# Tyler-Linchenwei/Graph-Distillation-for-Recommendation

Hardware: NVIDIA B200
Metric: kmeans_iters_per_s (higher is better)
Workload: dtype f32

## Files before the change

### graph-distillation-for-recommendation_b200/csrc/kmeans_tc.cu

```cuda
#include "tc_common.cuh"
#include <cuda.h>
#include <string.h>
#include <stdlib.h>

namespace gdr {

int launch_row_sqnorm(int64_t K, int D, const float* C, int64_t ldc, float* out, cudaStream_t s);
int launch_assign_simt_rows(int64_t max_rows, int64_t K, int64_t D, const float* X, int64_t ldx,
                            const float* CT, int64_t ldct, const float* cnorm, const int32_t* rows,
                            const int32_t* n_rows_dev, unsigned long long* packed, int32_t* labels,
                            const int32_t* labels_prev, int32_t* n_changed, float* best_out, cudaStream_t s);

constexpr int TC_BN = 128;
constexpr int TC_MAX_KB = 4;
constexpr int TC_BAR_KB = 5;
constexpr int TC_STAGES = 3;
constexpr int TC_THREADS = 320;
constexpr int TC_EPI_THREADS = 256;
constexpr int TC_TMEM_COLS = 256;
constexpr float TC_BAND = 3.0517578125e-05f;
static const int32_t* g_last_count1 = nullptr;
int g_tc_ablate = 0;
int g_tc_gate = 1;
extern int64_t g_topk_last_overflow;
// ... 780 lines not shown
          t1 = clock64();
          e_ld += t1 - t0;
        }
        tc_fence_before();
        mbar_arrive(&t_empty[a]);
        if (probe) e_ar += clock64() - t1;
      }
      if (half == 1) {
        s_merge[rl] = best;
        s_merge[128 + rl] = second;
        reinterpret_cast<int*>(s_merge)[256 + rl] = bidx;
      }
      asm volatile("bar.sync 1, %0;" ::"n"(TC_EPI_THREADS) : "memory");
      if (half == 0) {
        const float b1 = s_merge[rl], s1 = s_merge[128 + rl];
        const int i1 = reinterpret_cast<int*>(s_merge)[256 + rl];
        const float nb = fminf(best, b1);
        const float ns = fminf(fminf(second, s1), fmaxf(best, b1));
        const int ni = b1 < best ? i1 : bidx;
        if (row < N) {
          best_out[row] = nb;
          second_out[row] = ns;
          idx_out[row] = ni;
        }
      }
      asm volatile("bar.sync 1, %0;" ::"n"(TC_EPI_THREADS) : "memory");
    }
    if (probe && lane == 0) {
      g_ts_probe[7] = clock64() - e_tot;
      g_ts_probe[8] = e_wt;
      g_ts_probe[9] = e_ld;
      g_ts_probe[10] = e_ar;
      g_ts_probe[11] = e_st;
    }
  }
  tc_fence_before();
  __syncthreads();
  if (warp == 1) {
    __syncwarp();
    asm volatile("tcgen05.dealloc.cta_group::1.sync.aligned.b32 %0, %1;" ::"r"(tmem_base), "r"(512) : "memory");
  }
}

__device__ __forceinline__ uint32_t cluster_ctarank() {
  uint32_t r;
  asm volatile("mov.u32 %0, %%cluster_ctarank;" : "=r"(r));
  return r;
}
__device__ __forceinline__ void cluster_sync_all() {
  asm volatile("barrier.cluster.arrive.release.aligned;" ::: "memory");
  asm volatile("barrier.cluster.wait.acquire.aligned;" ::: "memory");
}
__device__ __forceinline__ uint32_t mapa_u32(uint32_t smem_addr, uint32_t cta_rank) {
  uint32_t r;
  asm volatile("mapa.shared::cluster.u32 %0, %1, %2;" : "=r"(r) : "r"(smem_addr), "r"(cta_rank));
  return r;
}
__device__ __forceinline__ void mbar_arrive_cluster(uint32_t cluster_addr) {
  asm volatile("mbarrier.arrive.release.cluster.shared::cluster.b64 _, [%0];" ::"r"(cluster_addr) : "memory");
}
__device__ __forceinline__ void tma_load_2d_2sm(void* smem_dst, const CUtensorMap* map, int c0, int c1,
                                                uint32_t bar_cluster_addr) {
  asm volatile(
      "cp.async.bulk.tensor.2d.cta_group::2.shared::cluster.global.mbarrier::complete_tx::bytes [%0], [%1, {%2, %3}], [%4];"
      ::"r"(smem_u32(smem_dst)), "l"(reinterpret_cast<uint64_t>(map)), "r"(c0), "r"(c1), "r"(bar_cluster_addr)
      : "memory");
}
__device__ __forceinline__ void tc_commit_2sm(uint64_t* bar, uint16_t cta_mask) {
  asm volatile(
      "tcgen05.commit.cta_group::2.mbarrier::arrive::one.shared::cluster.multicast::cluster.b64 [%0], %1;"
      ::"r"(smem_u32(bar)), "h"(cta_mask)
      : "memory");
}
__device__ __forceinline__ void tc_mma_tf32_2sm(uint32_t tmem_d, uint64_t adesc, uint64_t bdesc, uint32_t idesc,
                                                uint32_t accumulate) {
  asm volatile(
      "{\n\t.reg .pred p;\n\t"
      "setp.ne.b32 p, %4, 0;\n\t"
      "tcgen05.mma.cta_group::2.kind::tf32 [%0], %1, %2, %3, p;\n\t}"
      ::"r"(tmem_d), "l"(adesc), "l"(bdesc), "r"(idesc), "r"(accumulate)
      : "memory");
}

struct Tc2Cfg {
  static constexpr int BN = 256;
  static constexpr int kStageBytes = (BN / 2) * TC_BK * 4;
  static constexpr int kStages = 8;
  static constexpr int kTmemCols = 2 * BN;
  static constexpr int kTail = 512;
  __host__ __device__ static constexpr int x_blk(int kb) { return kb * TC_KBLK_BYTES; }
  __host__ __device__ static constexpr int c_stage(int nkb, int s) { return nkb * TC_KBLK_BYTES + s * kStageBytes; }
  __host__ __device__ static constexpr int bars(int nkb) { return c_stage(nkb, kStages); }
  __host__ __device__ static constexpr int total(int nkb) { return bars(nkb) + kTail + 1024; }
};

__global__ void __launch_bounds__(TC_THREADS, 1)
k_assign_tc_pair(const __grid_constant__ CUtensorMap map_x, const __grid_constant__ CUtensorMap map_c,
                 int64_t N_host, const int32_t* __restrict__ n_rows_dev, int D, int n_col_tiles, int nkb,
                 float* __restrict__ best_out, float* __restrict__ second_out, int32_t* __restrict__ idx_out, int ablate,
                 int fwd ) {
  using Cfg = Tc2Cfg;
  constexpr int S = Cfg::kStages;
  constexpr int BN = Cfg::BN;
  extern __shared__ uint8_t smem_raw[];
  uint8_t* smem = reinterpret_cast<uint8_t*>((reinterpret_cast<uintptr_t>(smem_raw) + 1023) & ~uintptr_t(1023));
  uint64_t* bars = reinterpret_cast<uint64_t*>(smem + Cfg::bars(nkb));
  uint64_t* x_full = bars;
  uint64_t* x_empty = bars + TC_BAR_KB;
  uint64_t* c_full = bars + 2 * TC_BAR_KB;
  uint64_t* c_empty = c_full + S;
  uint64_t* t_full = c_empty + S;
  uint64_t* t_empty = t_full + 2;
  uint64_t* c_peer = t_empty + 2;
  uint64_t* x_peer = c_peer + S;
  uint32_t* tmem_base_smem = reinterpret_cast<uint32_t*>(x_peer + TC_BAR_KB);

  const int warp = threadIdx.x >> 5;
  const int lane = threadIdx.x & 31;
  const uint32_t crank = cluster_ctarank();
  const bool leader = crank == 0;
  const int64_t N = n_rows_dev ? (int64_t)n_rows_dev[0] : N_host;
  const int n_row_tiles = (int)((N + TC_BM - 1) / TC_BM);
  const int n_units = (n_row_tiles + 1) / 2;
  const int unit0 = (int)blockIdx.x >> 1, unit_stride = (int)gridDim.x >> 1;

  if (warp == 0 && lane == 0) {
    for (int i = 0; i < TC_BAR_KB; ++i) {
      mbar_init(&x_full[i], 1);
      mbar_init(&x_empty[i], 1);
    }
    for (int i = 0; i < S; ++i) {
      mbar_init(&c_full[i], 1);
      mbar_init(&c_empty[i], 1);
    }
    for (int i = 0; i < 2; ++i) {
      mbar_init(&t_full[i], 1);
      mbar_init(&t_empty[i], 16);
    }
    for (int i = 0; i < S; ++i) mbar_init(&c_peer[i], 1);
    for (int i = 0; i < TC_BAR_KB; ++i) mbar_init(&x_peer[i], 1);
    asm volatile("fence.mbarrier_init.release.cluster;" ::: "memory");
  }
  if (warp == 1) {
    asm volatile("tcgen05.alloc.cta_group::2.sync.aligned.shared::cta.b32 [%0], %1;" ::"r"(smem_u32(tmem_base_smem)),
                 "r"(Cfg::kTmemCols)
                 : "memory");
    asm volatile("tcgen05.relinquish_alloc_permit.cta_group::2.sync.aligned;" ::: "memory");
  }
  tc_fence_before();
  __syncthreads();
  cluster_sync_all();
  tc_fence_after();
  const uint32_t tmem_base = *tmem_base_smem;

  if (warp == 0) {
    uint32_t tile_it = 0;
    int s = 0;
    uint32_t ph = 0;
    const uint32_t x_full0 = mapa_u32(smem_u32(&x_full[0]), 0), c_full0 = mapa_u32(smem_u32(&c_full[0]), 0);
    for (int un = unit0; un < n_units; un += unit_stride, ++tile_it) {
      const int rt = 2 * un + (int)crank;
      for (int kb = 0; kb < nkb; ++kb) {
        mbar_wait(&x_empty[kb], (tile_it & 1) ^ 1);
        if (elect_one()) {
          if (fwd) {
            mbar_expect_tx(&x_full[kb], TC_KBLK_BYTES);
            tma_load_2d(smem + Cfg::x_blk(kb), &map_x, kb * TC_BK, rt * TC_BM, &x_full[kb]);
          } else {
            if (leader) mbar_expect_tx(&x_full[kb], 2 * TC_KBLK_BYTES);
            tma_load_2d_2sm(smem + Cfg::x_blk(kb), &map_x, kb * TC_BK, rt * TC_BM, x_full0 + 8u * (uint32_t)kb);
          }
        }
        __syncwarp();
      }
      for (int ct = 0; ct < n_col_tiles; ++ct) {
        for (int kb = 0; kb < nkb; ++kb) {
          if (ablate >= 6) continue;
          mbar_wait(&c_empty[s], ph ^ 1);
          if (elect_one()) {
            if (ablate == 5) {
              if (leader || fwd) mbar_arrive(&c_full[s]);
            } else if (fwd) {
              mbar_expect_tx(&c_full[s], Cfg::kStageBytes);
              tma_load_2d(smem + Cfg::c_stage(nkb, s), &map_c, kb * TC_BK, ct * BN + (int)crank * (BN / 2), &c_full[s]);
            } else {
              if (leader) mbar_expect_tx(&c_full[s], 2 * Cfg::kStageBytes);
              tma_load_2d_2sm(smem + Cfg::c_stage(nkb, s), &map_c, kb * TC_BK, ct * BN + (int)crank * (BN / 2),
                              c_full0 + 8u * (uint32_t)s);
            }
          }
          __syncwarp();
          if (++s == S) {
            s = 0;
            ph ^= 1;
          }
        }
      }
    }
  } else if (warp == 1) {
    if (leader) {
      constexpr uint32_t idesc = umma_idesc_tf32(2 * TC_BM, BN);
      uint32_t tile_it = 0, g = 0;
      int s = 0;
      uint32_t ph = 0;
      const uint64_t dx0 = umma_desc_sw128(smem_u32(smem));
      const uint64_t dc0 = umma_desc_sw128(smem_u32(smem + Cfg::c_stage(nkb, 0)));
      constexpr uint64_t kKb = TC_KBLK_BYTES >> 4, kStage = Cfg::kStageBytes >> 4;
      for (int un = unit0; un < n_units; un += unit_stride, ++tile_it) {
        for (int ct = 0; ct < n_col_tiles; ++ct, ++g) {
          const uint32_t a = g & 1, aph = (g >> 1) & 1;
          if (ablate != 8) mbar_wait(&t_empty[a], aph ^ 1);
          tc_fence_after();
          const uint32_t tmem_d = tmem_base + a * BN;
          const bool last_ct = ct == n_col_tiles - 1;
          for (int kb = 0; kb < nkb; ++kb) {
            if (ct == 0) {
              mbar_wait(&x_full[kb], tile_it & 1);
              if (fwd) mbar_wait(&x_peer[kb], tile_it & 1);
            }
            if (ablate < 6) {
              mbar_wait(&c_full[s], ph);
              if (fwd) mbar_wait(&c_peer[s], ph);
            }
            tc_fence_after();
            const uint64_t d_x = dx0 + (uint64_t)kb * kKb;
            const uint64_t d_c = dc0 + (uint64_t)s * kStage;
            const int ksteps = min(TC_BK / 8, (D - kb * TC_BK + 7) >> 3);
            if (elect_one()) {
              if (ablate != 3 && ablate != 4 && ksteps == 4) {
#pragma unroll
                for (int k = 0; k < 4; ++k) {
                  const uint64_t adv = (uint64_t)((k * 8 * 4) >> 4);
                  tc_mma_tf32_2sm(tmem_d, d_x + adv, d_c + adv, idesc, (kb | k) != 0);
                }
              } else {
                for (int k = 0; k < ((ablate == 3 || (ablate == 4 && kb > 0)) ? 0 : ksteps); ++k) {
                  const uint64_t adv = (uint64_t)((k * 8 * 4) >> 4);
                  tc_mma_tf32_2sm(tmem_d, d_x + adv, d_c + adv, idesc, (kb | k) != 0);
                }
              }
              if (ablate < 6) tc_commit_2sm(&c_empty[s], 3);
              if (last_ct) tc_commit_2sm(&x_empty[kb], 3);
              if (kb == nkb - 1 && ablate != 8) tc_commit_2sm(&t_full[a], 3);
            }
            __syncwarp();
            if (++s == S) {
              s = 0;
              ph ^= 1;
            }
          }
        }
      }
    } else if (fwd) {
      uint32_t tile_it = 0;
      int s = 0;
      uint32_t ph = 0;
      const uint32_t c_peer0 = mapa_u32(smem_u32(&c_peer[0]), 0), x_peer0 = mapa_u32(smem_u32(&x_peer[0]), 0);
      for (int un = unit0; un < n_units; un += unit_stride, ++tile_it) {
        for (int ct = 0; ct < n_col_tiles; ++ct) {
          for (int kb = 0; kb < nkb; ++kb) {
            if (ct == 0) {
              mbar_wait(&x_full[kb], tile_it & 1);
              if (elect_one()) mbar_arrive_cluster(x_peer0 + 8u * (uint32_t)kb);
              __syncwarp();
            }
            mbar_wait(&c_full[s], ph);
            if (elect_one()) mbar_arrive_cluster(c_peer0 + 8u * (uint32_t)s);
            __syncwarp();
            if (++s == S) {
              s = 0;
              ph ^= 1;
            }
          }
        }
      }
    }
  } else {
    const int quarter = warp & 3;
    const int half = (warp - 2) >> 2;
    const int rl = quarter * 32 + lane;
    const uint32_t t_empty_leader[2] = {mapa_u32(smem_u32(&t_empty[0]), 0), mapa_u32(smem_u32(&t_empty[1]), 0)};
    __shared__ float s_mb[3][TC_BM];
    uint32_t g = 0;
    for (int un = unit0; un < (ablate == 8 ? 0 : n_units); un += unit_stride) {
      const int rt = 2 * un + (int)crank;
      const int64_t row = (int64_t)rt * TC_BM + rl;
      float best = INFINITY, second = INFINITY;
      int bidx = 0;
      for (int ct = 0; ct < n_col_tiles; ++ct, ++g) {
        const uint32_t a = g & 1, aph = (g >> 1) & 1;
        mbar_wait(&t_full[a], aph);
        tc_fence_after();
#pragma unroll 1
        for (int h2 = 0; h2 < (ablate == 2 ? 0 : BN / 128); ++h2) {
          const int col0 = half * (BN / 2) + h2 * 64;
          const uint32_t taddr = tmem_base + ((uint32_t)(quarter * 32) << 16) + a * BN + col0;
          uint32_t v[2][32];
          tc_ld_32x32(taddr, v[0]);
          tc_ld_32x32(taddr + 32, v[1]);
          tc_wait_ld();
#pragma unroll
          for (int c = 0; c < 2; ++c) {
            const int jbase = ct * BN + col0 + c * 32;
#pragma unroll
            for (int u0 = 0; u0 < 32; u0 += 8) {
              float m = fmaxf(fmaxf(__uint_as_float(v[c][u0]), __uint_as_float(v[c][u0 + 1])),
                              fmaxf(__uint_as_float(v[c][u0 + 2]), __uint_as_float(v[c][u0 + 3])));
              m = fmaxf(m, fmaxf(fmaxf(__uint_as_float(v[c][u0 + 4]), __uint_as_float(v[c][u0 + 5])),
                                 fmaxf(__uint_as_float(v[c][u0 + 6]), __uint_as_float(v[c][u0 + 7]))));
              if (__any_sync(0xffffffffu, -m < second)) {
#pragma unroll
                for (int u = u0; u < u0 + 8; ++u) {
                  const float d = -__uint_as_float(v[c][u]);
                  second = fminf(second, fmaxf(d, best));
                  bidx = d < best ? jbase + u : bidx;
                  best = fminf(best, d);
                }
              }
            }
          }
        }
        tc_fence_before();
        __syncwarp();
        if (lane == 0) mbar_arrive_cluster(t_empty_leader[a]);
      }
      if (half == 1) {
        s_mb[0][rl] = best;
        s_mb[1][rl] = second;
        reinterpret_cast<int*>(s_mb[2])[rl] = bidx;
      }
      asm volatile("bar.sync 1, %0;" ::"n"(TC_EPI_THREADS) : "memory");
      if (half == 0) {
        const float b1 = s_mb[0][rl], s1 = s_mb[1][rl];
        const int i1 = reinterpret_cast<int*>(s_mb[2])[rl];
        const float nb = fminf(best, b1);
        const float ns = fminf(fminf(second, s1), fmaxf(best, b1));
        const int ni = b1 < best ? i1 : bidx;
        if (row < N) {
          best_out[row] = nb;
          second_out[row] = ns;
          idx_out[row] = ni;
        }
      }
      asm volatile("bar.sync 1, %0;" ::"n"(TC_EPI_THREADS) : "memory");
    }
  }
  tc_fence_before();
  __syncthreads();
  cluster_sync_all();
  if (warp == 1) {
    asm volatile("tcgen05.dealloc.cta_group::2.sync.aligned.b32 %0, %1;" ::"r"(tmem_base), "r"(Cfg::kTmemCols) : "memory");
  }
}

__global__ void __launch_bounds__(128, 1) k_mma_probe_pair(int iters, long long* __restrict__ cycles) {
  extern __shared__ uint8_t smem_raw[];
  uint8_t* smem = reinterpret_cast<uint8_t*>((reinterpret_cast<uintptr_t>(smem_raw) + 1023) & ~uintptr_t(1023));
  __shared__ uint64_t bar;
  __shared__ uint32_t tmem_slot;
  for (int i = threadIdx.x; i < 8 * 128 * 128 / 4; i += blockDim.x) reinterpret_cast<float*>(smem)[i] = 0.f;
  const bool leader = cluster_ctarank() == 0;
  if (threadIdx.x == 0) {
    mbar_init(&bar, 1);
    asm volatile("fence.mbarrier_init.release.cluster;" ::: "memory");
  }
  if (threadIdx.x < 32) {
    asm volatile("tcgen05.alloc.cta_group::2.sync.aligned.shared::cta.b32 [%0], %1;" ::"r"(smem_u32(&tmem_slot)), "r"(512) : "memory");
    asm volatile("tcgen05.relinquish_alloc_permit.cta_group::2.sync.aligned;" ::: "memory");
  }
  asm volatile("fence.proxy.async.shared::cta;" ::: "memory");
  tc_fence_before();
  __syncthreads();
  cluster_sync_all();
  tc_fence_after();
  const uint32_t tmem_base = tmem_slot;
  if (leader && threadIdx.x < 32) {
    constexpr uint32_t idesc = umma_idesc_tf32(256, 256);
    const long long t0 = clock64();
    int issued = 0;
    for (int t = 0; issued < iters; ++t) {
      const uint32_t d = tmem_base + (uint32_t)(t & 1) * 256u;
      for (int kb = 0; kb < 4; ++kb) {
        const uint64_t da = umma_desc_sw128(smem_u32(smem + kb * 16384));
        const uint64_t db = umma_desc_sw128(smem_u32(smem + 65536 + ((t * 4 + kb) & 3) * 16384));
        const int ks = kb < 3 ? 4 : 1;
        tc_fence_after();
        if (elect_one()) {
          for (int k = 0; k < ks; ++k) {
            const uint64_t adv = (uint64_t)((k * 32) >> 4);
            tc_mma_tf32_2sm(d, da + adv, db + adv, idesc, (kb | k) != 0);
          }
        }
        __syncwarp();
        issued += ks;
      }
    }
    if (elect_one()) tc_commit_2sm(&bar, 1);
    __syncwarp();
    mbar_wait(&bar, 0);
    if (threadIdx.x == 0) cycles[0] = clock64() - t0;
  }
  tc_fence_before();
  __syncthreads();
  cluster_sync_all();
  if (threadIdx.x < 32) {
    asm volatile("tcgen05.dealloc.cta_group::2.sync.aligned.b32 %0, %1;" ::"r"(tmem_base), "r"(512) : "memory");
  }
}

__global__ void __launch_bounds__(256) k_tc_select1(int64_t N, const float* __restrict__ best,
                                                    const float* __restrict__ second,
                                                    const int32_t* __restrict__ idx,
                                                    const float* __restrict__ xnorm, const float* __restrict__ xdnorm,
                                                    const float* __restrict__ cnorm,
                                                    const float* __restrict__ cnorm_sqrt,
                                                    const float* __restrict__ cdnorm,
                                                    const float* __restrict__ cmax, float band,
// ... 418 lines not shown
         ws_need(2 * N, 4) + ws_need(2 * N * TC_CAND_CAP, 8)  + ws_need(N, 4)  +
         256  + 256;
}

template <int NPASS, int BN, int SUB>
static int launch_assign_tc(const CUtensorMap& m_xhi, const CUtensorMap& m_xlo, const CUtensorMap& m_chi,
                            const CUtensorMap& m_clo, int64_t N_max, const int32_t* n_rows_dev, int D_eff, int64_t Kp,
                            int nkb, const float* cnorm, float* best, float* second, int32_t* idx, cudaStream_t s,
                            TcGate gate = TcGate{nullptr, nullptr, nullptr, nullptr, 0.f}) {
  using Cfg = TcCfg<NPASS, BN, SUB>;
  static PerDevice<bool> attr_set_dev;
  bool& attr_set = attr_set_dev.get();
  if (!attr_set) {
    GDR_CUDA(cudaFuncSetAttribute(k_assign_tc<NPASS, BN, SUB>, cudaFuncAttributeMaxDynamicSharedMemorySize,
                                  TC_SMEM_LIMIT));
    attr_set = true;
  }
  int sms = kSMs;
  {
    int dev = 0;
    cudaGetDevice(&dev);
    cudaDeviceGetAttribute(&sms, cudaDevAttrMultiProcessorCount, dev);
  }
  const int64_t tiles = cdiv(N_max, TC_BM * SUB);
  const int grid = (int)(tiles < sms ? tiles : sms);
  k_assign_tc<NPASS, BN, SUB><<<grid, TC_THREADS, Cfg::total(nkb), s>>>(m_xhi, m_xlo, m_chi, m_clo, N_max, n_rows_dev, D_eff,
                                                                  (int)(Kp / BN), nkb, cnorm, best, second, idx, g_tc_ablate, gate);
  GDR_LAUNCHED();
  return GDR_OK;
}

static int launch_tc_cand(const CUtensorMap& m_x1, const CUtensorMap& m_c1, int64_t N_max, const int32_t* n_rows_dev,
                          int D_eff, int64_t Kp, int nkb, TcGate gate, TcCand cand, cudaStream_t s) {
  using Cfg = TcCfg<1, 256, 1>;
  static PerDevice<bool> attr_set_dev;
  bool& attr_set = attr_set_dev.get();
  if (!attr_set) {
    GDR_CUDA(cudaFuncSetAttribute(k_tc_cand, cudaFuncAttributeMaxDynamicSharedMemorySize, TC_SMEM_LIMIT));
    attr_set = true;
  }
  int sms = kSMs;
  {
    int dev = 0;
    cudaGetDevice(&dev);
    cudaDeviceGetAttribute(&sms, cudaDevAttrMultiProcessorCount, dev);
  }
  const int64_t tiles = cdiv(N_max, TC_BM);
  const int grid = (int)(tiles < sms ? tiles : sms);
  k_tc_cand<<<grid, TC_THREADS, Cfg::total(nkb), s>>>(m_x1, m_c1, N_max, n_rows_dev, D_eff, (int)(Kp / 256), nkb, gate, cand);
  GDR_LAUNCHED();
  return GDR_OK;
}

template <int BN>
static int launch_assign_tc_ts(const float* x1, int ldx1, const CUtensorMap& m_c, int64_t N_max, const int32_t* n_rows_dev,
                               int D_eff, int n_col_tiles, int nkb, float* best, float* second, int32_t* idx, cudaStream_t s,
                               TcGate gate) {
  using Cfg = TsCfg<BN>;
  static PerDevice<bool> attr_set_dev;
  bool& attr_set = attr_set_dev.get();
  if (!attr_set) {
    GDR_CUDA(cudaFuncSetAttribute(k_assign_tc_ts<BN>, cudaFuncAttributeMaxDynamicSharedMemorySize, TC_SMEM_LIMIT));
    attr_set = true;
  }
  int sms = kSMs;
  {
    int dev = 0;
    cudaGetDevice(&dev);
    cudaDeviceGetAttribute(&sms, cudaDevAttrMultiProcessorCount, dev);
  }
  const int64_t tiles = cdiv(N_max, TC_BM);
  const int grid = (int)(tiles < sms ? tiles : sms);
  k_assign_tc_ts<BN><<<grid, TC_THREADS, Cfg::total(), s>>>(x1, ldx1, m_c, N_max, n_rows_dev, D_eff, n_col_tiles, nkb, best,
                                                          second, idx, g_tc_ablate, gate);
  GDR_LAUNCHED();
  return GDR_OK;
}

__global__ void k_pad_aug(float* __restrict__ aug, int64_t r0, int64_t r1, int Dp1, int D) {
  const int64_t i = (int64_t)blockIdx.x * blockDim.x + threadIdx.x, n = (r1 - r0) * Dp1;
  if (i < n) aug[r0 * Dp1 + i] = (int)(i % Dp1) == D + 2 ? to_tf32(-1e30f) : 0.f;
}

static int launch_assign_tc_pair(const CUtensorMap& m_x, const CUtensorMap& m_c, int64_t N_max, const int32_t* n_rows_dev,
                                 int D_eff, int64_t Kp, int nkb, float* best, float* second, int32_t* idx, int fwd,
                                 cudaStream_t s) {
  static PerDevice<bool> attr_set_dev;
  bool& attr_set = attr_set_dev.get();
  if (!attr_set) {
    GDR_CUDA(cudaFuncSetAttribute(k_assign_tc_pair, cudaFuncAttributeMaxDynamicSharedMemorySize, Tc2Cfg::total(TC_BAR_KB)));
    attr_set = true;
  }
  int sms = kSMs;
  {
    int dev = 0;
    cudaGetDevice(&dev);
    cudaDeviceGetAttribute(&sms, cudaDevAttrMultiProcessorCount, dev);
  }
  const int64_t units = cdiv(cdiv(N_max, TC_BM), 2);
  const int pairs = (int)(units < sms / 2 ? units : sms / 2);
  cudaLaunchConfig_t cfg = {};
  cfg.gridDim = dim3(2 * pairs);
  cfg.blockDim = dim3(TC_THREADS);
  cfg.dynamicSmemBytes = Tc2Cfg::total(nkb);
  cfg.stream = s;
  cudaLaunchAttribute attr[1];
  attr[0].id = cudaLaunchAttributeClusterDimension;
  attr[0].val.clusterDim.x = 2;
  attr[0].val.clusterDim.y = 1;
  attr[0].val.clusterDim.z = 1;
  cfg.attrs = attr;
  cfg.numAttrs = 1;
  GDR_CUDA(cudaLaunchKernelEx(&cfg, k_assign_tc_pair, m_x, m_c, N_max, n_rows_dev, D_eff, (int)(Kp / Tc2Cfg::BN), nkb, best,
                              second, idx, g_tc_ablate, fwd));
  GDR_LAUNCHED();
  return GDR_OK;
}

int kmeans_assign_tc_run(int64_t N, int64_t K, int64_t D, const float* X, int64_t ldx, const void* xsplit,
                         const float* C, int64_t ldc, int32_t* labels, const int32_t* labels_prev,
                         int32_t* n_changed_dev, float* best_out, int32_t* n_refined_dev, void* ws,
                         int64_t ws_bytes, cudaStream_t s, const int32_t* labels_hint) {
  if (D > TC_MAX_KB * TC_BK) {
    set_error("kmeans_assign(tc): D=%lld > %d is not supported by the tensor-core path", (long long)D,
              TC_MAX_KB * TC_BK);
    return GDR_EUNSUPPORTED;
  }
  if (N >= (1ll << 31) - TC_BM || K >= (1ll << 31) - TC_KPAD) {
    set_error("kmeans_assign(tc): N or K exceeds int32 tile coordinates");
    return GDR_ERANGE;
  }
  const int Dp = dpad(D), Dp1 = dpad1(D);
  const int nkb = Dp / TC_BK, nkb1 = Dp1 / TC_BK;
  const int64_t Kp = align_up(K, TC_KPAD);
  XSplit xs = carve_xsplit(const_cast<void*>(xsplit), N, D);
  Workspace W(ws, ws_bytes);
  float* c_hi = W.take<float>(Kp * Dp);
  float* c_lo = W.take<float>(Kp * Dp);
  float* c_t = W.take<float>(Kp * Dp);
  float* c1 = W.take<float>((Kp + TC_TS_BN) * Dp1);
  float* cnorm = W.take<float>(Kp);
  float* cnorm_sqrt = W.take<float>(Kp);
  float* cdnorm = W.take<float>(Kp);
  float* cmax = W.take<float>(2);
  float* best = W.take<float>(N);
  float* second = W.take<float>(N);
  int32_t* idx = W.take<int32_t>(N);
  int32_t* amb_list = W.take<int32_t>(N);
  unsigned long long* amb_packed = W.take<unsigned long long>(N);
  int32_t* amb_count_ws = W.take<int32_t>(1);
  int32_t* list1 = W.take<int32_t>(N);
  int32_t* count1 = W.take<int32_t>(1);
  float* g_hi = W.take<float>(N * Dp);
  float* g_lo = W.take<float>(N * Dp);
  float* g_norm = W.take<float>(N);
  float* g_dnorm = W.take<float>(N);
  float* g_seed = W.take<float>(N);
  int32_t* cand_n = W.take<int32_t>(2 * N);
  int2* cand_list = W.take<int2>(2 * N * TC_CAND_CAP);
  int32_t* list2 = W.take<int32_t>(N);
  int32_t* cand_ctr = W.take<int32_t>(TC_CAND_CTRS);
  int32_t* amb_count = n_refined_dev ? n_refined_dev : amb_count_ws;
  if (!W.ok()) {
    set_error("kmeans_assign(tc): workspace too small");
    return GDR_EWORKSPACE;
  }
  const bool two_level = tc_two_level(N, best_out != nullptr);
  k_split_tf32<<<(unsigned)cdiv(Kp * 32, 256), 256, 0, s>>>(K, Kp, (int)D, Dp, C, ldc, c_hi, c_lo, nullptr, c_t, cnorm,
                                                           two_level ? c1 : nullptr, Dp1, 2, cdnorm);
  GDR_LAUNCHED();
  int rc;
  k_cnorm_finish<<<1, 1024, 0, s>>>(K, Kp, cnorm, two_level ? cdnorm : nullptr, cnorm_sqrt, cmax, amb_count, count1,
                                    two_level ? cand_ctr : nullptr, TC_CAND_CTRS);
  GDR_LAUNCHED();

  CUtensorMap m_xhi, m_xlo, m_chi, m_clo;
  if ((rc = make_map(&m_chi, c_hi, Kp, Dp, 128))) return rc;
  if ((rc = make_map(&m_clo, c_lo, Kp, Dp, 128))) return rc;

  if (!two_level) {
    if ((rc = make_map(&m_xhi, xs.hi, N, Dp, TC_BM))) return rc;
    if ((rc = make_map(&m_xlo, xs.lo, N, Dp, TC_BM))) return rc;
    {
      ProfileScope prof(PROF_ASSIGN, s);
      if ((rc = launch_assign_tc<3, 128, 1>(m_xhi, m_xlo, m_chi, m_clo, N, nullptr, (int)D, Kp, nkb, cnorm, best, second,
                                         idx, s)))
        return rc;
    }
    k_tc_select<<<(unsigned)cdiv(N, 256), 256, 0, s>>>(N, best, second, idx, xs.norm, cmax, TC_BAND, labels,
                                                      labels_prev, n_changed_dev, best_out, amb_list, amb_count,
                                                      amb_packed);
    GDR_LAUNCHED();
  } else {
    ProfileScope prof(PROF_ASSIGN, s);
    CUtensorMap m_x1, m_c1;
    bool cand_level = false;
    if ((rc = make_map(&m_x1, xs.x1, N, Dp1, TC_BM))) return rc;
    if (g_tc_screen == 2) {
      if ((rc = make_map(&m_c1, c1, Kp, Dp1, 128))) return rc;
      if ((rc = launch_assign_tc<1, 128, 2>(m_x1, m_x1, m_c1, m_c1, N, nullptr, (int)D + TC_AUG, Kp, nkb1, cnorm, best, second,
                                         idx, s)))
        return rc;
    } else if (g_tc_screen == 4 || g_tc_screen == 5) {
      if ((rc = make_map(&m_c1, c1, Kp, Dp1, 128))) return rc;
      if ((rc = launch_assign_tc_pair(m_x1, m_c1, N, nullptr, (int)D + TC_AUG, Kp, nkb1, best, second, idx,
                                      g_tc_screen == 5 ? 1 : 0, s)))
        return rc;
    } else {
      const int ka = (int)align_up(D + TC_AUG, 8);
      const int ts_bn = (g_tc_screen == 6 && ka <= 512 - 2 * TC_TS_BN) ? TC_TS_BN : 0;
      cand_level = g_tc_cand != 0 && ts_bn == 0;
      const int64_t k_rows = ts_bn == TC_TS_BN ? align_up(K, TC_TS_BN) : Kp;
      if (k_rows > Kp) {
        k_pad_aug<<<(unsigned)cdiv((k_rows - Kp) * Dp1, 256), 256, 0, s>>>(c1, Kp, k_rows, Dp1, (int)D);
        GDR_LAUNCHED();
      }
      if ((rc = make_map(&m_c1, c1, std::max(Kp, k_rows), Dp1, ts_bn ? ts_bn : 256))) return rc;
      TcGate gate{nullptr, nullptr, nullptr, nullptr, TC_BAND};
      if (g_tc_gate) {
        gate.xnorm = xs.norm;
        gate.xdnorm = xs.dnorm;
        gate.cscal = cmax;
        const int32_t* hint = labels_hint ? labels_hint : labels_prev;
        if (hint && g_tc_gate >= 2) {
          float* seed = g_norm;
          k_tc_seed<<<(unsigned)cdiv(N * 32, 256), 256, 0, s>>>(N, K, Dp1, xs.x1, c1, hint, xs.norm, cmax, seed);
          GDR_LAUNCHED();
          gate.seed = seed;
        }
      }
      if (ts_bn == TC_TS_BN)
        rc = launch_assign_tc_ts<TC_TS_BN>(xs.x1, Dp1, m_c1, N, nullptr, (int)D + TC_AUG, (int)(k_rows / TC_TS_BN), nkb1, best,
                                           second, idx, s, gate);
      else
        rc = launch_assign_tc<1, 256, 1>(m_x1, m_x1, m_c1, m_c1, N, nullptr, (int)D + TC_AUG, Kp, nkb1, cnorm, best, second,
                                         idx, s, gate);
      if (rc) return rc;
    }
    if (g_tc_ablate) return GDR_OK;
    g_last_count1 = count1;
    k_tc_select1<<<(unsigned)cdiv(N, 256), 256, 0, s>>>(N, best, second, idx, xs.norm, xs.dnorm, cnorm, cnorm_sqrt,
                                                       cdnorm, cmax, TC_BAND, labels, labels_prev, n_changed_dev,
                                                       list1, count1);
    GDR_LAUNCHED();
    const int32_t* list_f = list1;
    const int32_t* count_f = count1;
    g_last_cand = cand_level ? cand_ctr : nullptr;
    if (cand_level) {
      float* g_x1 = g_hi;
      k_tc_gather_cand<<<4 * kSMs, 256, 0, s>>>(list1, count1, Dp1, xs.x1, xs.norm, xs.dnorm, best, g_x1, g_norm, g_dnorm,
                                                g_seed);
      GDR_LAUNCHED();
      CUtensorMap m_gx1;
      if ((rc = make_map(&m_gx1, g_x1, N, Dp1, TC_BM))) return rc;
      const int cap = g_tc_cand_cap > 0 ? std::min(g_tc_cand_cap, TC_CAND_CAP) : TC_CAND_CAP;
      if ((rc = launch_tc_cand(m_gx1, m_c1, N, count1, (int)D + TC_AUG, Kp, nkb1, TcGate{g_norm, g_dnorm, cmax, g_seed, TC_BAND},
                               TcCand{cand_list, cand_n, cap}, s)))
        return rc;
      k_tc_cand_resolve<<<4 * kSMs, 256, 0, s>>>(list1, count1, cand_list, cand_n, cap, g_seed, g_norm, g_dnorm, (int)D, X, ldx,
                                                 C, ldc, cnorm, cnorm_sqrt, cdnorm, cmax, TC_BAND, labels, labels_prev,
                                                 n_changed_dev, list2, cand_ctr);
      GDR_LAUNCHED();
      list_f = list2;
      count_f = cand_ctr;
    }
    k_tc_gather<<<4 * kSMs, 256, 0, s>>>(list_f, count_f, Dp, xs.hi, xs.lo, xs.norm, g_hi, g_lo, g_norm);
    GDR_LAUNCHED();
    CUtensorMap m_ghi, m_glo;
    if ((rc = make_map(&m_ghi, g_hi, N, Dp, TC_BM))) return rc;
    if ((rc = make_map(&m_glo, g_lo, N, Dp, TC_BM))) return rc;
    if ((rc = launch_assign_tc<3, 128, 1>(m_ghi, m_glo, m_chi, m_clo, N, count_f, (int)D, Kp, nkb, cnorm, best, second, idx,
                                       s)))
      return rc;
    k_tc_select2<<<2 * kSMs, 256, 0, s>>>(list_f, count_f, best, second, idx, g_norm, cmax, TC_BAND, labels,
                                         labels_prev, n_changed_dev, amb_list, amb_count, amb_packed);
    GDR_LAUNCHED();
  }
  rc = launch_assign_simt_rows(N, K, D, X, ldx, c_t, Kp, cnorm, amb_list, amb_count, amb_packed, labels, labels_prev,
                               n_changed_dev, best_out, s);
  if (rc || !two_level || !g_last_cand || !n_refined_dev) return rc;
  k_add_i32<<<1, 1, 0, s>>>(n_refined_dev, cand_ctr + 1);
  GDR_LAUNCHED();
  return GDR_OK;
}

int64_t kmeans_assign_tc_total_ws_bytes(int64_t N, int64_t K, int64_t D) {
  return kmeans_assign_tc_ws_bytes(N, K, D) + kmeans_tc_xsplit_bytes(N, D);
}

int kmeans_assign_tc(int64_t N, int64_t K, int64_t D, const float* X, int64_t ldx, const float* C, int64_t ldc,
                     int32_t* labels, const int32_t* labels_prev, int32_t* n_changed_dev, float* best_out,
                     void* ws, int64_t ws_bytes, cudaStream_t s) {
  if (ws_bytes < kmeans_assign_tc_total_ws_bytes(N, K, D)) {
    set_error("kmeans_assign(tc): workspace too small");
    return GDR_EWORKSPACE;
  }
  char* xsplit = (char*)ws + kmeans_assign_tc_ws_bytes(N, K, D);
  int rc = kmeans_tc_prepare(N, D, X, ldx, xsplit, s);
  if (rc) return rc;
  return kmeans_assign_tc_run(N, K, D, X, ldx, xsplit, C, ldc, labels, labels_prev, n_changed_dev, best_out,
                              nullptr, ws, kmeans_assign_tc_ws_bytes(N, K, D), s, nullptr);
}

}

extern "C" {

int gdr_debug_get(const char* key, int64_t* value_host) {
  GDR_CHECK_ARG(key && value_host, "debug_get: bad arguments");
  if (!strncmp(key, "ts_probe_", 9)) {
    long long h[16];
    GDR_CUDA(cudaMemcpyFromSymbol(h, gdr::g_ts_probe, sizeof(h)));
    const int i = atoi(key + 9);
    GDR_CHECK_ARG(i >= 0 && i < 16, "debug_get: ts_probe index");
// ... 108 lines not shown
```

### graph-distillation-for-recommendation_b200/csrc/tc_common.cuh

```cuda
#pragma once
#include "common.cuh"
#include <cuda.h>

namespace gdr {

constexpr int TC_BM = 128;
constexpr int TC_BK = 32;
constexpr int TC_KBLK_BYTES = TC_BM * TC_BK * 4;

__device__ __forceinline__ uint32_t smem_u32(const void* p) {
  return (uint32_t)__cvta_generic_to_shared(p);
}
__device__ __forceinline__ void mbar_init(uint64_t* bar, uint32_t count) {
  asm volatile("mbarrier.init.shared::cta.b64 [%0], %1;" ::"r"(smem_u32(bar)), "r"(count) : "memory");
}
__device__ __forceinline__ void mbar_expect_tx(uint64_t* bar, uint32_t bytes) {
  asm volatile("mbarrier.arrive.expect_tx.shared::cta.b64 _, [%0], %1;" ::"r"(smem_u32(bar)), "r"(bytes)
               : "memory");
}
__device__ __forceinline__ void mbar_arrive(uint64_t* bar) {
  asm volatile("mbarrier.arrive.shared::cta.b64 _, [%0];" ::"r"(smem_u32(bar)) : "memory");
}
__device__ __forceinline__ void mbar_wait(uint64_t* bar, uint32_t parity) {
  uint32_t addr = smem_u32(bar), ok;
  do {
    asm volatile(
        "{\n\t.reg .pred p;\n\t"
        "mbarrier.try_wait.parity.shared::cta.b64 p, [%1], %2;\n\t"
        "selp.u32 %0, 1, 0, p;\n\t}"
        : "=r"(ok)
        : "r"(addr), "r"(parity)
        : "memory");
  } while (!ok);
}
__device__ __forceinline__ bool elect_one() {
  uint32_t pred = 0;
  asm volatile(
      "{\n\t.reg .pred p;\n\t"
      "elect.sync _|p, 0xffffffff;\n\t"
      "selp.u32 %0, 1, 0, p;\n\t}"
      : "=r"(pred));
  return pred != 0;
}
__device__ __forceinline__ void tma_load_2d(void* smem_dst, const CUtensorMap* map, int c0, int c1,
                                            uint64_t* bar) {
  asm volatile(
      "cp.async.bulk.tensor.2d.shared::cluster.global.mbarrier::complete_tx::bytes [%0], [%1, {%2, %3}], [%4];"
      ::"r"(smem_u32(smem_dst)), "l"(reinterpret_cast<uint64_t>(map)), "r"(c0), "r"(c1), "r"(smem_u32(bar))
      : "memory");
}
__device__ __forceinline__ void tc_fence_before() { asm volatile("tcgen05.fence::before_thread_sync;" ::: "memory"); }
__device__ __forceinline__ void tc_fence_after() { asm volatile("tcgen05.fence::after_thread_sync;" ::: "memory"); }
__device__ __forceinline__ void tc_commit(uint64_t* bar) {
  asm volatile("tcgen05.commit.cta_group::1.mbarrier::arrive::one.shared::cluster.b64 [%0];" ::"r"(smem_u32(bar))
               : "memory");
}
__device__ __forceinline__ void tc_mma_tf32(uint32_t tmem_d, uint64_t adesc, uint64_t bdesc, uint32_t idesc,
                                            uint32_t accumulate) {
  asm volatile(
      "{\n\t.reg .pred p;\n\t"
      "setp.ne.b32 p, %4, 0;\n\t"
      "tcgen05.mma.cta_group::1.kind::tf32 [%0], %1, %2, %3, p;\n\t}"
      ::"r"(tmem_d), "l"(adesc), "l"(bdesc), "r"(idesc), "r"(accumulate)
      : "memory");
}
__device__ __forceinline__ void tc_mma_bf16(uint32_t tmem_d, uint64_t adesc, uint64_t bdesc, uint32_t idesc,
                                            uint32_t accumulate) {
  asm volatile(
      "{\n\t.reg .pred p;\n\t"
      "setp.ne.b32 p, %4, 0;\n\t"
      "tcgen05.mma.cta_group::1.kind::f16 [%0], %1, %2, %3, p;\n\t}"
      ::"r"(tmem_d), "l"(adesc), "l"(bdesc), "r"(idesc), "r"(accumulate)
      : "memory");
}
__device__ __forceinline__ void tc_ld_32x32(uint32_t taddr, uint32_t (&v)[32]) {
  asm volatile(
      "tcgen05.ld.sync.aligned.32x32b.x32.b32 "
      "{%0, %1, %2, %3, %4, %5, %6, %7, %8, %9, %10, %11, %12, %13, %14, %15, "
      "%16, %17, %18, %19, %20, %21, %22, %23, %24, %25, %26, %27, %28, %29, %30, %31}, [%32];"
      : "=r"(v[0]), "=r"(v[1]), "=r"(v[2]), "=r"(v[3]), "=r"(v[4]), "=r"(v[5]), "=r"(v[6]), "=r"(v[7]),
        "=r"(v[8]), "=r"(v[9]), "=r"(v[10]), "=r"(v[11]), "=r"(v[12]), "=r"(v[13]), "=r"(v[14]), "=r"(v[15]),
        "=r"(v[16]), "=r"(v[17]), "=r"(v[18]), "=r"(v[19]), "=r"(v[20]), "=r"(v[21]), "=r"(v[22]), "=r"(v[23]),
        "=r"(v[24]), "=r"(v[25]), "=r"(v[26]), "=r"(v[27]), "=r"(v[28]), "=r"(v[29]), "=r"(v[30]), "=r"(v[31])
      : "r"(taddr)
      : "memory");
}
__device__ __forceinline__ void tc_wait_ld() { asm volatile("tcgen05.wait::ld.sync.aligned;" ::: "memory"); }

__device__ __forceinline__ uint64_t umma_desc_sw128(uint32_t smem_addr) {
  uint64_t d = 0;
  d |= (uint64_t)((smem_addr & 0x3FFFF) >> 4);
  d |= (uint64_t)1 << 16;
  d |= (uint64_t)(1024 >> 4) << 32;
  d |= (uint64_t)1 << 46;
  d |= (uint64_t)2 << 61;
  return d;
}
__host__ __device__ constexpr uint32_t umma_idesc_tf32(int M, int N) {
  return (1u << 4) | (2u << 7) | (2u << 10) | ((uint32_t)(N >> 3) << 17) | ((uint32_t)(M >> 4) << 24);
}

__device__ __forceinline__ float to_tf32(float x) {
  uint32_t u;
  asm("cvt.rna.tf32.f32 %0, %1;" : "=r"(u) : "f"(x));
  return __uint_as_float(u);
}

typedef CUresult (*PFN_tmapEncodeTiled)(CUtensorMap*, CUtensorMapDataType, cuuint32_t, void*, const cuuint64_t*,
                                        const cuuint64_t*, const cuuint32_t*, const cuuint32_t*,
                                        CUtensorMapInterleave, CUtensorMapSwizzle, CUtensorMapL2promotion,
                                        CUtensorMapFloatOOBfill);

static PFN_tmapEncodeTiled get_encode() {
  static PFN_tmapEncodeTiled fn = nullptr;
  if (!fn) {
    void* p = nullptr;
    cudaDriverEntryPointQueryResult q;
    if (cudaGetDriverEntryPoint("cuTensorMapEncodeTiled", &p, cudaEnableDefault, &q) == cudaSuccess &&
        q == cudaDriverEntryPointSuccess)
      fn = (PFN_tmapEncodeTiled)p;
  }
  return fn;
}

static int make_map(CUtensorMap* m, const float* base, int64_t rows, int Dp, int box_rows) {
  PFN_tmapEncodeTiled enc = get_encode();
  if (!enc) {
    set_error("cuTensorMapEncodeTiled entry point not available");
    return GDR_ECUDA;
  }
  cuuint64_t gdim[2] = {(cuuint64_t)Dp, (cuuint64_t)rows};
  cuuint64_t gstr[1] = {(cuuint64_t)Dp * 4};
  cuuint32_t box[2] = {(cuuint32_t)TC_BK, (cuuint32_t)box_rows};
  cuuint32_t estr[2] = {1, 1};
  CUresult r = enc(m, CU_TENSOR_MAP_DATA_TYPE_FLOAT32, 2, (void*)base, gdim, gstr, box, estr,
                   CU_TENSOR_MAP_INTERLEAVE_NONE, CU_TENSOR_MAP_SWIZZLE_128B, CU_TENSOR_MAP_L2_PROMOTION_L2_256B,
                   CU_TENSOR_MAP_FLOAT_OOB_FILL_NONE);
  if (r != CUDA_SUCCESS) {
    set_error("cuTensorMapEncodeTiled failed with %d", (int)r);
    return GDR_ECUDA;
  }
  return GDR_OK;
}

}
```

Before: 97.79.

## Route default TC screen to 2-SM pair kernel with narrow K-tail and gating

Makes the 2-CTA cluster tcgen05 pair kernel the default assignment path when the augmented dimension fits, instead of only under screens 4/5. The last K block can now be loaded and multiplied with a narrow 32B/64B swizzled tile, which avoids moving and computing padding columns. Pipeline stage count now comes from the shared memory left over, up to 12 instead of a fixed 8. The epilogue gains chunk skipping and norm-based candidate gating. This adds complexity in descriptor and swizzle handling and makes correctness depend on the gating tolerance.

Result: slower. 93.47 (median of 6 runs) (-4.4%).

```diff
diff --git a/graph-distillation-for-recommendation_b200/csrc/kmeans_tc.cu b/graph-distillation-for-recommendation_b200/csrc/kmeans_tc.cu
--- a/graph-distillation-for-recommendation_b200/csrc/kmeans_tc.cu
+++ b/graph-distillation-for-recommendation_b200/csrc/kmeans_tc.cu
@@ -886,38 +886,54 @@
       : "memory");
 }
 
+__host__ __device__ constexpr int tc_tail_cols(int D_eff, int nkb) {
+  return ((D_eff - (nkb - 1) * TC_BK + 7) & ~7) <= 16 ? ((D_eff - (nkb - 1) * TC_BK + 7) & ~7) : TC_BK;
+}
+
 struct Tc2Cfg {
   static constexpr int BN = 256;
   static constexpr int kStageBytes = (BN / 2) * TC_BK * 4;
-  static constexpr int kStages = 8;
+  static constexpr int kMaxStages = 12;
   static constexpr int kTmemCols = 2 * BN;
-  static constexpr int kTail = 512;
+  static constexpr int kTail = 512  + 1536 ;
   __host__ __device__ static constexpr int x_blk(int kb) { return kb * TC_KBLK_BYTES; }
-  __host__ __device__ static constexpr int c_stage(int nkb, int s) { return nkb * TC_KBLK_BYTES + s * kStageBytes; }
-  __host__ __device__ static constexpr int bars(int nkb) { return c_stage(nkb, kStages); }
-  __host__ __device__ static constexpr int total(int nkb) { return bars(nkb) + kTail + 1024; }
+  __host__ __device__ static constexpr int x_bytes(int nkb, int tail) { return (nkb - 1) * TC_KBLK_BYTES + TC_BM * tail * 4; }
+  __host__ __device__ static constexpr int c_stage(int nkb, int tail, int s) {
+    return ((x_bytes(nkb, tail) + 1023) & ~1023) + s * kStageBytes;
+  }
+  __host__ __device__ static constexpr int stages(int nkb, int tail) {
+    int n = (TC_SMEM_LIMIT - 1024  - kTail - c_stage(nkb, tail, 0)) / kStageBytes;
+    return n > kMaxStages ? kMaxStages : n;
+  }
+  __host__ __device__ static constexpr int bars(int nkb, int tail) { return c_stage(nkb, tail, stages(nkb, tail)); }
+  __host__ __device__ static constexpr int total(int nkb, int tail) { return bars(nkb, tail) + kTail + 1024; }
 };
 
 __global__ void __launch_bounds__(TC_THREADS, 1)
 k_assign_tc_pair(const __grid_constant__ CUtensorMap map_x, const __grid_constant__ CUtensorMap map_c,
+                 const __grid_constant__ CUtensorMap map_xt, const __grid_constant__ CUtensorMap map_ct,
+                 int tail ,
                  int64_t N_host, const int32_t* __restrict__ n_rows_dev, int D, int n_col_tiles, int nkb,
                  float* __restrict__ best_out, float* __restrict__ second_out, int32_t* __restrict__ idx_out, int ablate,
-                 int fwd ) {
+                 int fwd ,
+                 TcGate gate) {
   using Cfg = Tc2Cfg;
-  constexpr int S = Cfg::kStages;
+  constexpr int SM = Cfg::kMaxStages;
+  const int S = Cfg::stages(nkb, tail);
   constexpr int BN = Cfg::BN;
   extern __shared__ uint8_t smem_raw[];
   uint8_t* smem = reinterpret_cast<uint8_t*>((reinterpret_cast<uintptr_t>(smem_raw) + 1023) & ~uintptr_t(1023));
-  uint64_t* bars = reinterpret_cast<uint64_t*>(smem + Cfg::bars(nkb));
+  uint64_t* bars = reinterpret_cast<uint64_t*>(smem + Cfg::bars(nkb, tail));
   uint64_t* x_full = bars;
   uint64_t* x_empty = bars + TC_BAR_KB;
   uint64_t* c_full = bars + 2 * TC_BAR_KB;
-  uint64_t* c_empty = c_full + S;
-  uint64_t* t_full = c_empty + S;
+  uint64_t* c_empty = c_full + SM;
+  uint64_t* t_full = c_empty + SM;
   uint64_t* t_empty = t_full + 2;
   uint64_t* c_peer = t_empty + 2;
-  uint64_t* x_peer = c_peer + S;
+  uint64_t* x_peer = c_peer + SM;
   uint32_t* tmem_base_smem = reinterpret_cast<uint32_t*>(x_peer + TC_BAR_KB);
+  float* s_merge = reinterpret_cast<float*>(reinterpret_cast<uint8_t*>(bars) + 512);
 
   const int warp = threadIdx.x >> 5;
   const int lane = threadIdx.x & 31;
@@ -933,7 +949,7 @@
       mbar_init(&x_full[i], 1);
       mbar_init(&x_empty[i], 1);
     }
-    for (int i = 0; i < S; ++i) {
+    for (int i = 0; i < SM; ++i) {
       mbar_init(&c_full[i], 1);
       mbar_init(&c_empty[i], 1);
     }
@@ -941,7 +957,7 @@
       mbar_init(&t_full[i], 1);
       mbar_init(&t_empty[i], 16);
     }
-    for (int i = 0; i < S; ++i) mbar_init(&c_peer[i], 1);
+    for (int i = 0; i < SM; ++i) mbar_init(&c_peer[i], 1);
     for (int i = 0; i < TC_BAR_KB; ++i) mbar_init(&x_peer[i], 1);
     asm volatile("fence.mbarrier_init.release.cluster;" ::: "memory");
   }
@@ -967,12 +983,15 @@
       for (int kb = 0; kb < nkb; ++kb) {
         mbar_wait(&x_empty[kb], (tile_it & 1) ^ 1);
         if (elect_one()) {
+          const bool tl = kb == nkb - 1 && tail < TC_BK;
+          const CUtensorMap* mx = tl ? &map_xt : &map_x;
+          const uint32_t bytes = tl ? TC_BM * tail * 4 : TC_KBLK_BYTES;
           if (fwd) {
-            mbar_expect_tx(&x_full[kb], TC_KBLK_BYTES);
-            tma_load_2d(smem + Cfg::x_blk(kb), &map_x, kb * TC_BK, rt * TC_BM, &x_full[kb]);
+            mbar_expect_tx(&x_full[kb], bytes);
+            tma_load_2d(smem + Cfg::x_blk(kb), mx, kb * TC_BK, rt * TC_BM, &x_full[kb]);
           } else {
-            if (leader) mbar_expect_tx(&x_full[kb], 2 * TC_KBLK_BYTES);
-            tma_load_2d_2sm(smem + Cfg::x_blk(kb), &map_x, kb * TC_BK, rt * TC_BM, x_full0 + 8u * (uint32_t)kb);
+            if (leader) mbar_expect_tx(&x_full[kb], 2 * bytes);
+            tma_load_2d_2sm(smem + Cfg::x_blk(kb), mx, kb * TC_BK, rt * TC_BM, x_full0 + 8u * (uint32_t)kb);
           }
         }
         __syncwarp();
@@ -982,14 +1001,17 @@
           if (ablate >= 6) continue;
           mbar_wait(&c_empty[s], ph ^ 1);
           if (elect_one()) {
+            const bool tl = kb == nkb - 1 && tail < TC_BK;
+            const CUtensorMap* mc = tl ? &map_ct : &map_c;
+            const uint32_t bytes = tl ? (BN / 2) * tail * 4 : Cfg::kStageBytes;
             if (ablate == 5) {
               if (leader || fwd) mbar_arrive(&c_full[s]);
             } else if (fwd) {
-              mbar_expect_tx(&c_full[s], Cfg::kStageBytes);
-              tma_load_2d(smem + Cfg::c_stage(nkb, s), &map_c, kb * TC_BK, ct * BN + (int)crank * (BN / 2), &c_full[s]);
+              mbar_expect_tx(&c_full[s], bytes);
+              tma_load_2d(smem + Cfg::c_stage(nkb, tail, s), mc, kb * TC_BK, ct * BN + (int)crank * (BN / 2), &c_full[s]);
             } else {
-              if (leader) mbar_expect_tx(&c_full[s], 2 * Cfg::kStageBytes);
-              tma_load_2d_2sm(smem + Cfg::c_stage(nkb, s), &map_c, kb * TC_BK, ct * BN + (int)crank * (BN / 2),
+              if (leader) mbar_expect_tx(&c_full[s], 2 * bytes);
+              tma_load_2d_2sm(smem + Cfg::c_stage(nkb, tail, s), mc, kb * TC_BK, ct * BN + (int)crank * (BN / 2),
                               c_full0 + 8u * (uint32_t)s);
             }
           }
@@ -1008,7 +1030,9 @@
       int s = 0;
       uint32_t ph = 0;
       const uint64_t dx0 = umma_desc_sw128(smem_u32(smem));
-      const uint64_t dc0 = umma_desc_sw128(smem_u32(smem + Cfg::c_stage(nkb, 0)));
+      const uint64_t dc0 = umma_desc_sw128(smem_u32(smem + Cfg::c_stage(nkb, tail, 0)));
+      const uint64_t dxt0 = umma_desc_kmajor(smem_u32(smem), 4 * tail);
+      const uint64_t dct0 = umma_desc_kmajor(smem_u32(smem + Cfg::c_stage(nkb, tail, 0)), 4 * tail);
       constexpr uint64_t kKb = TC_KBLK_BYTES >> 4, kStage = Cfg::kStageBytes >> 4;
       for (int un = unit0; un < n_units; un += unit_stride, ++tile_it) {
         for (int ct = 0; ct < n_col_tiles; ++ct, ++g) {
@@ -1027,8 +1051,9 @@
               if (fwd) mbar_wait(&c_peer[s], ph);
             }
             tc_fence_after();
-            const uint64_t d_x = dx0 + (uint64_t)kb * kKb;
-            const uint64_t d_c = dc0 + (uint64_t)s * kStage;
+            const bool tl = kb == nkb - 1;
+            const uint64_t d_x = (tl ? dxt0 : dx0) + (uint64_t)kb * kKb;
+            const uint64_t d_c = (tl ? dct0 : dc0) + (uint64_t)s * kStage;
             const int ksteps = min(TC_BK / 8, (D - kb * TC_BK + 7) >> 3);
             if (elect_one()) {
               if (ablate != 3 && ablate != 4 && ksteps == 4) {
@@ -1084,13 +1109,22 @@
     const int half = (warp - 2) >> 2;
     const int rl = quarter * 32 + lane;
     const uint32_t t_empty_leader[2] = {mapa_u32(smem_u32(&t_empty[0]), 0), mapa_u32(smem_u32(&t_empty[1]), 0)};
-    __shared__ float s_mb[3][TC_BM];
+    const bool chunk_skip = n_col_tiles * BN >= 4096;
+    const bool gated = chunk_skip && gate.xnorm != nullptr;
     uint32_t g = 0;
     for (int un = unit0; un < (ablate == 8 ? 0 : n_units); un += unit_stride) {
       const int rt = 2 * un + (int)crank;
       const int64_t row = (int64_t)rt * TC_BM + rl;
       float best = INFINITY, second = INFINITY;
       int bidx = 0;
+      float tolmax = 0.f, limt = INFINITY;
+      if (gated) {
+        const float xn = row < N ? gate.xnorm[row] : 0.f, xd = row < N ? gate.xdnorm[row] : 0.f;
+        const float cm = gate.cscal[0], cdm = gate.cscal[1];
+        tolmax = 1.001f * (2.02f * (xd * cm + xn * (cdm + 3.0517578125e-05f * cm) + 1.52587890625e-05f * cm * cm) +
+                           gate.band * xn * cm + 9.5367431640625e-07f * (xn * cm + cm * cm));
+        if (gate.seed != nullptr && row < N) limt = gate.seed[row] + tolmax;
+      }
       for (int ct = 0; ct < n_col_tiles; ++ct, ++g) {
         const uint32_t a = g & 1, aph = (g >> 1) & 1;
         mbar_wait(&t_full[a], aph);
@@ -1103,40 +1137,27 @@
           tc_ld_32x32(taddr, v[0]);
           tc_ld_32x32(taddr + 32, v[1]);
           tc_wait_ld();
-#pragma unroll
-          for (int c = 0; c < 2; ++c) {
-            const int jbase = ct * BN + col0 + c * 32;
-#pragma unroll
-            for (int u0 = 0; u0 < 32; u0 += 8) {
-              float m = fmaxf(fmaxf(__uint_as_float(v[c][u0]), __uint_as_float(v[c][u0 + 1])),
-                              fmaxf(__uint_as_float(v[c][u0 + 2]), __uint_as_float(v[c][u0 + 3])));
-              m = fmaxf(m, fmaxf(fmaxf(__uint_as_float(v[c][u0 + 4]), __uint_as_float(v[c][u0 + 5])),
-                                 fmaxf(__uint_as_float(v[c][u0 + 6]), __uint_as_float(v[c][u0 + 7]))));
-              if (__any_sync(0xffffffffu, -m < second)) {
-#pragma unroll
-                for (int u = u0; u < u0 + 8; ++u) {
-                  const float d = -__uint_as_float(v[c][u]);
-                  second = fminf(second, fmaxf(d, best));
-                  bidx = d < best ? jbase + u : bidx;
-                  best = fminf(best, d);
-                }
-              }
-            }
-          }
+          if (ablate == 1) {
+            if (v[0][0] == 0x7fc12345u && v[1][31] == 0x7fc54321u) bidx = 1;
+            continue;
+          }
+#pragma unroll
+          for (int c = 0; c < 2; ++c)
+            epi_chunk32(v[c], ct * BN + col0 + c * 32, chunk_skip, gated, tolmax, limt, best, second, bidx);
         }
         tc_fence_before();
         __syncwarp();
         if (lane == 0) mbar_arrive_cluster(t_empty_leader[a]);
       }
       if (half == 1) {
-        s_mb[0][rl] = best;
-        s_mb[1][rl] = second;
-        reinterpret_cast<int*>(s_mb[2])[rl] = bidx;
+        s_merge[rl] = best;
+        s_merge[128 + rl] = second;
+        reinterpret_cast<int*>(s_merge)[256 + rl] = bidx;
       }
       asm volatile("bar.sync 1, %0;" ::"n"(TC_EPI_THREADS) : "memory");
       if (half == 0) {
-        const float b1 = s_mb[0][rl], s1 = s_mb[1][rl];
-        const int i1 = reinterpret_cast<int*>(s_mb[2])[rl];
+        const float b1 = s_merge[rl], s1 = s_merge[128 + rl];
+        const int i1 = reinterpret_cast<int*>(s_merge)[256 + rl];
         const float nb = fminf(best, b1);
         const float ns = fminf(fminf(second, s1), fmaxf(best, b1));
         const int ni = b1 < best ? i1 : bidx;
@@ -1721,13 +1742,13 @@
   if (i < n) aug[r0 * Dp1 + i] = (int)(i % Dp1) == D + 2 ? to_tf32(-1e30f) : 0.f;
 }
 
-static int launch_assign_tc_pair(const CUtensorMap& m_x, const CUtensorMap& m_c, int64_t N_max, const int32_t* n_rows_dev,
-                                 int D_eff, int64_t Kp, int nkb, float* best, float* second, int32_t* idx, int fwd,
-                                 cudaStream_t s) {
+static int launch_assign_tc_pair(const CUtensorMap& m_x, const CUtensorMap& m_c, const CUtensorMap& m_xt,
+                                 const CUtensorMap& m_ct, int64_t N_max, const int32_t* n_rows_dev, int D_eff, int64_t Kp,
+                                 int nkb, float* best, float* second, int32_t* idx, int fwd, cudaStream_t s, TcGate gate) {
   static PerDevice<bool> attr_set_dev;
   bool& attr_set = attr_set_dev.get();
   if (!attr_set) {
-    GDR_CUDA(cudaFuncSetAttribute(k_assign_tc_pair, cudaFuncAttributeMaxDynamicSharedMemorySize, Tc2Cfg::total(TC_BAR_KB)));
+    GDR_CUDA(cudaFuncSetAttribute(k_assign_tc_pair, cudaFuncAttributeMaxDynamicSharedMemorySize, TC_SMEM_LIMIT));
     attr_set = true;
   }
   int sms = kSMs;
@@ -1741,7 +1762,8 @@
   cudaLaunchConfig_t cfg = {};
   cfg.gridDim = dim3(2 * pairs);
   cfg.blockDim = dim3(TC_THREADS);
-  cfg.dynamicSmemBytes = Tc2Cfg::total(nkb);
+  const int tail = tc_tail_cols(D_eff, nkb);
+  cfg.dynamicSmemBytes = Tc2Cfg::total(nkb, tail);
   cfg.stream = s;
   cudaLaunchAttribute attr[1];
   attr[0].id = cudaLaunchAttributeClusterDimension;
@@ -1750,8 +1772,8 @@
   attr[0].val.clusterDim.z = 1;
   cfg.attrs = attr;
   cfg.numAttrs = 1;
-  GDR_CUDA(cudaLaunchKernelEx(&cfg, k_assign_tc_pair, m_x, m_c, N_max, n_rows_dev, D_eff, (int)(Kp / Tc2Cfg::BN), nkb, best,
-                              second, idx, g_tc_ablate, fwd));
+  GDR_CUDA(cudaLaunchKernelEx(&cfg, k_assign_tc_pair, m_x, m_c, m_xt, m_ct, tail, N_max, n_rows_dev, D_eff,
+                              (int)(Kp / Tc2Cfg::BN), nkb, best, second, idx, g_tc_ablate, fwd, gate));
   GDR_LAUNCHED();
   return GDR_OK;
 }
@@ -1840,14 +1862,10 @@
       if ((rc = launch_assign_tc<1, 128, 2>(m_x1, m_x1, m_c1, m_c1, N, nullptr, (int)D + TC_AUG, Kp, nkb1, cnorm, best, second,
                                          idx, s)))
         return rc;
-    } else if (g_tc_screen == 4 || g_tc_screen == 5) {
-      if ((rc = make_map(&m_c1, c1, Kp, Dp1, 128))) return rc;
-      if ((rc = launch_assign_tc_pair(m_x1, m_c1, N, nullptr, (int)D + TC_AUG, Kp, nkb1, best, second, idx,
-                                      g_tc_screen == 5 ? 1 : 0, s)))
-        return rc;
     } else {
       const int ka = (int)align_up(D + TC_AUG, 8);
       const int ts_bn = (g_tc_screen == 6 && ka <= 512 - 2 * TC_TS_BN) ? TC_TS_BN : 0;
+      const bool pair = (g_tc_screen == 0 || g_tc_screen == 4 || g_tc_screen == 5) && Dp1 <= TC_MAX_KB * TC_BK;
       cand_level = g_tc_cand != 0 && ts_bn == 0;
       const int64_t k_rows = ts_bn == TC_TS_BN ? align_up(K, TC_TS_BN) : Kp;
       if (k_rows > Kp) {
@@ -1868,7 +1886,15 @@
           gate.seed = seed;
         }
       }
-      if (ts_bn == TC_TS_BN)
+      if (pair) {
+        const int tail = tc_tail_cols((int)D + TC_AUG, nkb1);
+        CUtensorMap m_c1p, m_x1t, m_c1t;
+        if ((rc = make_map(&m_c1p, c1, Kp, Dp1, 128))) return rc;
+        if ((rc = make_map(&m_x1t, xs.x1, N, Dp1, TC_BM, tail))) return rc;
+        if ((rc = make_map(&m_c1t, c1, Kp, Dp1, 128, tail))) return rc;
+        rc = launch_assign_tc_pair(m_x1, m_c1p, m_x1t, m_c1t, N, nullptr, (int)D + TC_AUG, Kp, nkb1, best, second, idx,
+                                   g_tc_screen == 5 ? 1 : 0, s, gate);
+      } else if (ts_bn == TC_TS_BN)
         rc = launch_assign_tc_ts<TC_TS_BN>(xs.x1, Dp1, m_c1, N, nullptr, (int)D + TC_AUG, (int)(k_rows / TC_TS_BN), nkb1, best,
                                            second, idx, s, gate);
       else
diff --git a/graph-distillation-for-recommendation_b200/csrc/tc_common.cuh b/graph-distillation-for-recommendation_b200/csrc/tc_common.cuh
--- a/graph-distillation-for-recommendation_b200/csrc/tc_common.cuh
+++ b/graph-distillation-for-recommendation_b200/csrc/tc_common.cuh
@@ -87,15 +87,16 @@
 }
 __device__ __forceinline__ void tc_wait_ld() { asm volatile("tcgen05.wait::ld.sync.aligned;" ::: "memory"); }
 
-__device__ __forceinline__ uint64_t umma_desc_sw128(uint32_t smem_addr) {
+__device__ __forceinline__ uint64_t umma_desc_kmajor(uint32_t smem_addr, int sw_bytes) {
   uint64_t d = 0;
   d |= (uint64_t)((smem_addr & 0x3FFFF) >> 4);
   d |= (uint64_t)1 << 16;
-  d |= (uint64_t)(1024 >> 4) << 32;
+  d |= (uint64_t)((8 * sw_bytes) >> 4) << 32;
   d |= (uint64_t)1 << 46;
-  d |= (uint64_t)2 << 61;
+  d |= (uint64_t)(sw_bytes == 128 ? 2 : (sw_bytes == 64 ? 4 : 6)) << 61;
   return d;
 }
+__device__ __forceinline__ uint64_t umma_desc_sw128(uint32_t smem_addr) { return umma_desc_kmajor(smem_addr, 128); }
 __host__ __device__ constexpr uint32_t umma_idesc_tf32(int M, int N) {
   return (1u << 4) | (2u << 7) | (2u << 10) | ((uint32_t)(N >> 3) << 17) | ((uint32_t)(M >> 4) << 24);
 }
@@ -123,7 +124,7 @@
   return fn;
 }
 
-static int make_map(CUtensorMap* m, const float* base, int64_t rows, int Dp, int box_rows) {
+static int make_map(CUtensorMap* m, const float* base, int64_t rows, int Dp, int box_rows, int box_cols = TC_BK) {
   PFN_tmapEncodeTiled enc = get_encode();
   if (!enc) {
     set_error("cuTensorMapEncodeTiled entry point not available");
@@ -131,10 +132,12 @@
   }
   cuuint64_t gdim[2] = {(cuuint64_t)Dp, (cuuint64_t)rows};
   cuuint64_t gstr[1] = {(cuuint64_t)Dp * 4};
-  cuuint32_t box[2] = {(cuuint32_t)TC_BK, (cuuint32_t)box_rows};
+  cuuint32_t box[2] = {(cuuint32_t)box_cols, (cuuint32_t)box_rows};
   cuuint32_t estr[2] = {1, 1};
+  const CUtensorMapSwizzle sw = box_cols == TC_BK ? CU_TENSOR_MAP_SWIZZLE_128B
+                                : (box_cols == 16 ? CU_TENSOR_MAP_SWIZZLE_64B : CU_TENSOR_MAP_SWIZZLE_32B);
   CUresult r = enc(m, CU_TENSOR_MAP_DATA_TYPE_FLOAT32, 2, (void*)base, gdim, gstr, box, estr,
-                   CU_TENSOR_MAP_INTERLEAVE_NONE, CU_TENSOR_MAP_SWIZZLE_128B, CU_TENSOR_MAP_L2_PROMOTION_L2_256B,
+                   CU_TENSOR_MAP_INTERLEAVE_NONE, sw, CU_TENSOR_MAP_L2_PROMOTION_L2_256B,
                    CU_TENSOR_MAP_FLOAT_OOB_FILL_NONE);
   if (r != CUDA_SUCCESS) {
     set_error("cuTensorMapEncodeTiled failed with %d", (int)r);
```
